# WangXinyan940/openmm-chargeflux

Measured on AMD Instinct MI355X. Metric: ns/day + ms/force-eval, periodic charge-flux box, 1/2/4/8 MI355X, higher is better.
Workload: dtype f64; 1 GPU; C3: periodic flexible charge-flux water box, 96000 atoms, Ewald rc=1.0 nm tol=0.0001 (alpha 2.91842, kmax 31, K_half 113490), velocity Verlet dt=1 fs, fp64; atoms=96000, k_half=113490, handover=event, variants=0, kspace=grid (ES kernel W=13, pruned DFT), same k-set, parallelism=atom-decomposition x1

## Files before the change

include/chargeflux.h:

```cpp
#ifndef CHARGEFLUX_H_
#define CHARGEFLUX_H_

#include <stdint.h>

#ifdef __cplusplus
extern "C" {
#endif

#if defined(_WIN32)
#define CF_EXPORT __declspec(dllexport)
#else
#define CF_EXPORT __attribute__((visibility("default")))
#endif

#define CF_API_VERSION 4

#define CF_OK 0
#define CF_ERR_INVALID -1
#define CF_ERR_HIP -2
#define CF_ERR_STATE -3
#define CF_ERR_NOMEM -4

#define CF_ONE_4PI_EPS0 138.935456
#define CF_ONE_4PI_EPS0_CODATA2018 138.93545764438198
// ... 26 lines not shown

typedef struct cf_options {
    int32_t device;
    void* stream;
    int32_t rank;
    int32_t world_size;
    int32_t kspace_algo;
    int32_t grid_width;
    int32_t precision;
    int32_t handover;
    int32_t pair_list;
    int32_t variants;
    int32_t list_capacity;
    int32_t reserved[1];
} cf_options;

#define CF_PRECISION_DOUBLE 0
#define CF_PRECISION_MIXED 1

#define CF_HANDOVER_EVENT 0
#define CF_HANDOVER_MEMORY 1

#define CF_PAIR_LIST_AUTO 0
#define CF_PAIR_LIST_CLUSTER 1
#define CF_PAIR_LIST_ATOM_HALF 2
#define CF_PAIR_LIST_FULL 3

#define CF_VARIANT_GEMM_DFT 1
#define CF_VARIANT_VECTOR_SPREAD 2
#define CF_VARIANT_MFMA_SPREAD 4
#define CF_VARIANT_INTERP1 8
#define CF_VARIANT_INTERP2 16
#define CF_VARIANT_BLOCK_ROUNDS(r) (((r) & 15) << 8)

#define CF_INCLUDE_FORCES 1
#define CF_INCLUDE_ENERGY 2

typedef struct cf_handle cf_handle;

CF_EXPORT int cf_api_version(void);
CF_EXPORT const char* cf_last_error(void);

CF_EXPORT int cf_create(const cf_params* params, const cf_options* options, cf_handle** out);
CF_EXPORT int cf_destroy(cf_handle* h);

CF_EXPORT int cf_get_ewald_params(const cf_handle* h, double* alpha, int32_t kmax[3]);
CF_EXPORT int cf_get_grid_shape(const cf_handle* h, int32_t ng[3], int32_t* width);
CF_EXPORT int cf_get_owned_range(const cf_handle* h, int32_t* lo, int32_t* hi);
CF_EXPORT int cf_partition(const cf_params* params, int32_t world_size, int32_t rank, int32_t* lo, int32_t* hi);

CF_EXPORT int cf_set_neighbor_skin(cf_handle* h, double skin);
CF_EXPORT int cf_update_parameters(cf_handle* h, const cf_params* params);
CF_EXPORT int cf_get_pair_list(const cf_handle* h, int32_t* kind);
CF_EXPORT int cf_get_neighbor_stats(const cf_handle* h, int64_t* builds, int64_t* evaluations);
#define CF_FALLBACK_WINDOW 1
#define CF_FALLBACK_LIST 2
#define CF_FALLBACK_FIXED_POINT 4
CF_EXPORT int cf_get_fallback_stats(const cf_handle* h, int64_t* half_list_fallbacks, int64_t* rows_rescanned,
                                    int32_t* reasons);

#define CF_GUARD_CELL_BOUNDS 1
#define CF_GUARD_CLUSTER_TABLE 2
#define CF_GUARD_LIST_ENTRY 4
#define CF_GUARD_GRID_BINS 8
#define CF_GUARD_NEIGHBOR 16
#define CF_GUARD_ATOM_INDEX 32
// ... 42 lines not shown
```

openmm-chargeflux_amd/csrc/cf_api.hip:

```cpp
#include <hip/hip_runtime.h>

#include <algorithm>
#include <cmath>
#include <cstring>
#include <exception>
#include <numeric>
#include <stdexcept>
#include <string>
#include <vector>

#include "cf_internal.h"

enum Phase { PH_FLUX, PH_PREP, PH_CELLS, PH_NLIST, PH_TABLES, PH_SFAC, PH_COEFFS, PH_FORCE, PH_DIRECT,
             PH_ASSEMBLE, PH_ENERGY, PH_GSORT, PH_GSPREAD, PH_GDFTF, PH_GDFTI, PH_GINTERP, PH_EXCL, PH_COUNT };
static const char* kPhaseNames[PH_COUNT] = {"flux_terms", "atoms_prep", "cell_sort", "neighbor_list",
                                            "kspace_tables", "kspace_sfac", "kspace_coeffs", "kspace_force",
                                            "direct_pairs", "assemble", "energy", "grid_sort", "grid_spread",
                                            "grid_dft_fwd", "grid_dft_inv", "grid_interp", "direct_excl"};
constexpr int kMaxTimed = 8192;

static void graph_forget(cf_handle* H);
static void graph_invalidate(cf_handle* H);
struct GraphCache;
static GraphCache* graph_active(cf_handle* H);
// ... 408 lines not shown
        if (!p || !out) fail(CF_ERR_INVALID, "null argument");
        const int n = p->num_particles;
        if (n <= 0) fail(CF_ERR_INVALID, "num_particles must be > 0");
        if (!p->charges || !p->sigmas || !p->epsilons) fail(CF_ERR_INVALID, "particle arrays are null");
        cf_options o;
        std::memset(&o, 0, sizeof(o));
        if (opt) o = *opt;
        int world = o.world_size <= 1 ? 1 : o.world_size;
        if (o.rank < 0 || o.rank >= world) fail(CF_ERR_INVALID, "rank out of range");

        int ndev = 0;
        check_hip(hipGetDeviceCount(&ndev), "hipGetDeviceCount");
        if (ndev <= 0) fail(CF_ERR_HIP, "no HIP device available");
        if (o.device < 0 || o.device >= ndev) fail(CF_ERR_INVALID, "device ordinal out of range");
        check_hip(hipSetDevice(o.device), "hipSetDevice");

        H = new cf_handle();
        cf::Handle& h = H->h;
        h.n = n;
        h.device = o.device;
        h.rank = o.rank;
        h.world = world;
        if (o.kspace_algo < 0 || o.kspace_algo > 2) fail(CF_ERR_INVALID, "kspace_algo must be 0, 1 or 2");
        if (o.grid_width != 0 && (o.grid_width < 4 || o.grid_width > 16))
            fail(CF_ERR_INVALID, "grid_width must be 0 (default) or in [4, 16]");
        if (o.precision != CF_PRECISION_DOUBLE && o.precision != CF_PRECISION_MIXED)
            fail(CF_ERR_INVALID, "precision must be CF_PRECISION_DOUBLE or CF_PRECISION_MIXED");
        h.mixed = o.precision == CF_PRECISION_MIXED;
        if (o.handover != CF_HANDOVER_EVENT && o.handover != CF_HANDOVER_MEMORY)
            fail(CF_ERR_INVALID, "handover must be CF_HANDOVER_EVENT or CF_HANDOVER_MEMORY");
        if (o.pair_list < CF_PAIR_LIST_AUTO || o.pair_list > CF_PAIR_LIST_FULL)
            fail(CF_ERR_INVALID, "pair_list must be one of CF_PAIR_LIST_AUTO, _CLUSTER, _ATOM_HALF, _FULL "
                                 "(the octant list of API 3 was removed in API 4)");
        if (o.variants & ~(0x1F | (15 << 8))) fail(CF_ERR_INVALID, "unknown bits in variants");
        if (o.list_capacity < 0) fail(CF_ERR_INVALID, "list_capacity must be >= 0");
        h.handover_memory = o.handover == CF_HANDOVER_MEMORY;
        h.pair_list = o.pair_list;
        h.variants = o.variants;
        h.list_capacity = o.list_capacity;
        h.kspace_algo = o.kspace_algo;
        h.stream = (hipStream_t)o.stream;

        std::vector<double> q0;
        std::vector<double2> lj;
        parse_particles(p, q0, lj);

        const int B = p->num_flux_bonds, A = p->num_flux_angles, W = p->num_flux_waters;
        const int T = B + A + W;
        std::vector<int4> tidx;
        std::vector<double> tpar;
        std::vector<std::vector<int>> term_atoms;
        parse_terms(p, tidx, tpar, &term_atoms);
        H->topo_terms = tidx;
        h.nb = B; h.na = A; h.nw = W; h.nterms = T;
        h.nslots_dq = 2 * B + 3 * A + 3 * W;
        h.nd = 4 * B + 9 * A + 9 * W;
        std::vector<int> slot_atom(h.nslots_dq);
        {
            int s = 0;
            for (int t = 0; t < T; t++)
                for (int a : term_atoms[t]) slot_atom[s++] = a;
        }
        std::vector<int> qs(n + 1, 0), qslot(h.nslots_dq);
        for (int s = 0; s < h.nslots_dq; s++) qs[slot_atom[s] + 1]++;
        for (int i = 0; i < n; i++) qs[i + 1] += qs[i];
        {
            std::vector<int> fill(qs.begin(), qs.end() - 1);
// ... 372 lines not shown
    const bool reusable = h.pbc && h.skin > 0 && h.list_valid && s_call == h.list_skin &&
                          h.list_L[0] == h.box_L[0] && h.list_L[1] == h.box_L[1] && h.list_L[2] == h.box_L[2] &&
                          h.list_T[0] == h.box_t[0] && h.list_T[1] == h.box_t[1] && h.list_T[2] == h.box_t[2];
    if (h.pbc && !reusable) {
        h.list_skin = s_call;
        set_cells(H, h.box_L);
        h.list_valid = h.skin > 0;
        std::copy(h.box_L, h.box_L + 3, h.list_L);
        std::copy(h.box_t, h.box_t + 3, h.list_T);
    }
    h.n_evals++;
    return reusable;
}

static void launch_begin(cf_handle* H, const double* pos_dev, int flags, bool reusable) {
    cf::Handle& h = H->h;
    const int forces = flags & CF_INCLUDE_FORCES, energy = flags & CF_INCLUDE_ENERGY;
    { Timed t(H, PH_FLUX); cf::launch_flux_terms(h, pos_dev); }
    { Timed t(H, PH_PREP); cf::launch_atoms_prep(h, pos_dev, reusable); }
    if (h.pbc) {
        {
            Timed t(H, PH_CELLS);
            if (!reusable) cf::launch_force_rebuild(h);
            cf::launch_cell_sort(h, pos_dev);
        }
        if (h.hi > h.lo) { Timed t(H, PH_NLIST); cf::launch_nlist(h, pos_dev); }
        if ((forces || energy) && h.hi > h.lo) {
            if (h.kspace_algo == 0) {
                { Timed t(H, PH_TABLES); cf::launch_kspace_tables(h, pos_dev); }
                { Timed t(H, PH_SFAC); cf::launch_kspace_sfac(h); }
            } else if (h.kspace_algo == 2) {
                { Timed t(H, PH_GSORT); cf::launch_grid_sort(h, pos_dev); }
                { Timed t(H, PH_GSPREAD); cf::launch_grid_spread(h); }
                { Timed t(H, PH_GDFTF); cf::launch_grid_dft_fwd(h); }
            } else {
                Timed t(H, PH_SFAC);
                cf::launch_kspace_direct_sfac(h, pos_dev);
            }
        } else if (forces || energy) {
            int64_t cnt = 0;
            double* buf = cf::kspace_reduce_buffer(h, &cnt);
            cf::launch_zero(h, buf, cnt);
            if (h.kspace_algo == 1) cf::launch_kspace_kvec(h);
        }
    }
}

static void launch_direct(cf_handle* H) {
    cf::Handle& h = H->h;
    if (h.hi <= h.lo) return;
    const int flags = h.pending_flags;
    const int forces = flags & CF_INCLUDE_FORCES, energy = flags & CF_INCLUDE_ENERGY;
    if (h.pbc) {
        { Timed t(H, PH_DIRECT); cf::launch_direct(h, H->pos_pending, forces); }
        { Timed t(H, PH_EXCL); cf::launch_direct_finish(h, H->pos_pending, forces); }
    } else {
        Timed t(H, PH_DIRECT);
        cf::launch_nopbc(h, H->pos_pending, forces, energy);
    }
}

static void launch_end(cf_handle* H, int flags, double* forces_dev, double* energy_dev) {
    cf::Handle& h = H->h;
    const int forces = flags & CF_INCLUDE_FORCES, energy = flags & CF_INCLUDE_ENERGY;
    const double* pos = H->pos_pending;
    if (h.pbc && (forces || energy) && (h.hi > h.lo || h.rank == 0)) {
        Timed t(H, PH_COEFFS);
// ... 103 lines not shown
        (void)hipGraphDestroy(graph);
        check_hip(e, "hipGraphInstantiate");
        g->exec[seg] = ex;
        g->key[seg] = k;
        g->rec_split[seg] = h.rec_split;
        g->captures++;
    } else {
        h.rec_split = g->rec_split[seg];
        g->replays++;
    }
    check_hip(hipGraphLaunch(g->exec[seg], h.stream), "hipGraphLaunch");
}

extern "C" {
static GraphKey make_key(const cf::Handle& h, const void* pos, void* frc, void* ene, int flags, bool reusable,
                         const double* box9) {
    GraphKey k;
    k.pos = pos; k.frc = frc; k.ene = ene; k.flags = flags; k.reusable = reusable;
    k.epoch = h.alloc_epoch;
    if (h.pbc && box9) std::memcpy(k.box, box9, sizeof(k.box));
    return k;
}

static bool overlap_ok(const cf::Handle& h, int flags) {
    return h.overlap && h.aux && h.world == 1 && h.pbc && h.kspace_algo == 2 && h.hi > h.lo &&
           (flags & (CF_INCLUDE_FORCES | CF_INCLUDE_ENERGY));
}

static void launch_prologue(cf_handle* H, const double* pos_dev, bool reusable) {
    cf::Handle& h = H->h;
    { Timed t(H, PH_FLUX); cf::launch_flux_terms(h, pos_dev); }
    { Timed t(H, PH_PREP); cf::launch_atoms_prep(h, pos_dev, reusable); }
}
static void launch_direct_chain(cf_handle* H, const double* pos_dev, int flags, bool reusable) {
    cf::Handle& h = H->h;
    {
        Timed t(H, PH_CELLS);
        if (!reusable) cf::launch_force_rebuild(h);
        cf::launch_cell_sort(h, pos_dev);
    }
    { Timed t(H, PH_NLIST); cf::launch_nlist(h, pos_dev); }
    h.pending_flags = flags;
    launch_direct(H);
    h.pending_flags = -1;
}
static void launch_rec_fwd(cf_handle* H, const double* pos_dev) {
    cf::Handle& h = H->h;
    { Timed t(H, PH_GSORT); cf::launch_grid_sort(h, pos_dev); }
    { Timed t(H, PH_GSPREAD); cf::launch_grid_spread(h); }
    { Timed t(H, PH_GDFTF); cf::launch_grid_dft_fwd(h); }
}
static void launch_rec_end(cf_handle* H, int flags) {
    cf::Handle& h = H->h;
    { Timed t(H, PH_COEFFS); cf::launch_grid_coeffs(h, flags & CF_INCLUDE_ENERGY, (flags & CF_INCLUDE_FORCES) != 0); }
    if (flags & CF_INCLUDE_FORCES) {
        { Timed t(H, PH_GDFTI); cf::launch_grid_dft_inv(h); }
        { Timed t(H, PH_GINTERP); cf::launch_grid_interp(h, true); }
    }
}
}
template <class F>
static void on_aux(cf_handle* H, GraphCache* g, int seg, const GraphKey& k, F&& launches) {
    cf::Handle& h = H->h;
    const hipStream_t main = h.stream;
    h.stream = h.aux;
    try {
        run_segment(H, g, seg, k, launches);
    } catch (...) {
        h.stream = main;
        throw;
    }
    h.stream = main;
}
extern "C" {
static void fork_aux(cf::Handle& h) {
    check_hip(hipEventRecord(h.ev_fork, h.stream), "hipEventRecord (fork)");
    check_hip(hipStreamWaitEvent(h.aux, h.ev_fork, 0), "hipStreamWaitEvent (fork)");
}
static void wait_fork(cf::Handle& h) {
    check_hip(hipStreamWaitValue64(h.aux, h.sync_flag, ++h.sync_seq, hipStreamWaitValueGte, ~0ull),
              "hipStreamWaitValue64 (fork)");
}
static void join_post(cf::Handle& h) {
// ... 40 lines not shown
    size_t nd = 0;
    check_hip(hipStreamGetCaptureInfo_v2(cap, &st, &id, &graph, &deps, &nd), "hipStreamGetCaptureInfo_v2");
    if (st != hipStreamCaptureStatusActive || !graph) fail(CF_ERR_STATE, "capture_event_wait: stream is not capturing");
    std::vector<hipGraphNode_t> dep(deps, deps + nd);
    hipGraphNode_t w = nullptr;
    check_hip(hipGraphAddEventWaitNode(&w, graph, dep.empty() ? nullptr : dep.data(), dep.size(), ev),
              "hipGraphAddEventWaitNode");
    check_hip(hipStreamUpdateCaptureDependencies(cap, &w, 1, hipStreamSetCaptureDependencies),
              "hipStreamUpdateCaptureDependencies");
}

static void launch_full(cf_handle* H, const double* pos_dev, int flags, bool reusable, double* forces_dev,
                        double* energy_dev, GraphCache* g, const double* box9) {
    cf::Handle& h = H->h;
    struct Restore {
        cf::Handle& h; hipStream_t s;
        ~Restore() { h.pending_flags = -1; h.stream = s; }
    } restore{h, h.stream};
    if (!overlap_ok(h, flags)) {
        auto one = [&] {
            h.rec_split = false;
            h.pending_flags = flags;
            launch_begin(H, pos_dev, flags, reusable);
            launch_direct(H);
            h.pending_flags = -1;
            launch_end(H, flags, forces_dev, energy_dev);
        };
        run_segment(H, g, SEG_FULL, make_key(h, pos_dev, forces_dev, energy_dev, flags, reusable, box9), one);
        return;
    }
    const int forces = flags & CF_INCLUDE_FORCES, energy = flags & CF_INCLUDE_ENERGY;
    const GraphKey key = make_key(h, pos_dev, nullptr, nullptr, flags, reusable, box9);
    auto rec = [&] {
        launch_rec_fwd(H, pos_dev);
        launch_rec_end(H, flags);
    };
    auto dch = [&] { launch_direct_chain(H, pos_dev, flags, reusable); };
    if (h.handover_memory) {
        SyncGuard sync_guard{h};
        run_segment(H, g, SEG_PRO, key, [&] {
            launch_prologue(H, pos_dev, reusable);
            cf::launch_signal(h, h.sync_flag);
            rec();
        });
        wait_fork(h);
        on_aux(H, g, SEG_DCH, key, [&] {
            dch();
            cf::launch_signal(h, h.sync_flag + 1);
        });
        join_wait(h);
    } else {
        launch_prologue(H, pos_dev, reusable);
        fork_aux(h);
        on_aux(H, g, SEG_DCH, key, dch);
        join_post(h);
        if (g) {
            const GraphKey key_rec = make_key(h, pos_dev, forces_dev, energy_dev, flags, reusable, box9);
            run_segment(H, g, SEG_REC, key_rec, [&] {
                rec();
                capture_event_wait(h.stream, h.ev_join);
                h.rec_split = forces != 0;
                cf::launch_assemble_energy(h, (forces && forces_dev) ? forces_dev : nullptr, energy, energy_dev);
            });
            h.rec_split = forces != 0;
            return;
        }
        run_segment(H, g, SEG_REC, key, rec);
        join_wait(h);
    }
    h.rec_split = forces != 0;
    Timed t(H, PH_ENERGY);
    cf::launch_assemble_energy(h, (forces && forces_dev) ? forces_dev : nullptr, energy, energy_dev);
}

static bool split_overlap_ok(cf_handle* H, int flags) {
    const cf::Handle& h = H->h;
    return h.overlap && h.aux && h.world > 1 && h.pbc && h.kspace_algo == 2 && h.hi > h.lo &&
           (flags & (CF_INCLUDE_FORCES | CF_INCLUDE_ENERGY));
}

static void launch_begin_split(cf_handle* H, const double* pos_dev, int flags, bool reusable, GraphCache* g,
                               const double* box9) {
    cf::Handle& h = H->h;
    const GraphKey key = make_key(h, pos_dev, nullptr, nullptr, flags, reusable, box9);
    if (h.handover_memory) {
        SyncGuard sync_guard{h};
        run_segment(H, g, SEG_PRO, key, [&] {
            launch_prologue(H, pos_dev, reusable);
            cf::launch_signal(h, h.sync_flag);
            launch_rec_fwd(H, pos_dev);
        });
        wait_fork(h);
        try {
            on_aux(H, g, SEG_DCH, key, [&] {
                launch_direct_chain(H, pos_dev, flags, reusable);
                cf::launch_signal(h, h.sync_flag + 1);
            });
        } catch (...) {
            h.pending_flags = -1;
            throw;
        }
        return;
    }
    run_segment(H, g, SEG_PRO, key, [&] { launch_prologue(H, pos_dev, reusable); });
    fork_aux(h);
    try {
        on_aux(H, g, SEG_DCH, key, [&] { launch_direct_chain(H, pos_dev, flags, reusable); });
    } catch (...) {
        h.pending_flags = -1;
        throw;
    }
    join_post(h);
    run_segment(H, g, SEG_RFWD, key, [&] { launch_rec_fwd(H, pos_dev); });
}

static void launch_end_split(cf_handle* H, int flags, double* forces_dev, double* energy_dev, GraphCache* g,
                             const double* box9) {
    cf::Handle& h = H->h;
    const int forces = flags & CF_INCLUDE_FORCES, energy = flags & CF_INCLUDE_ENERGY;
    SyncGuard sync_guard{h};
    run_segment(H, g, SEG_REND, make_key(h, H->pos_pending, nullptr, nullptr, flags, false, box9),
                [&] { launch_rec_end(H, flags); });
    join_wait(h);
    h.rec_split = forces != 0;
    {
        Timed t(H, PH_ENERGY);
        cf::launch_assemble_energy(h, (forces && forces_dev) ? forces_dev : nullptr, energy, energy_dev);
    }
}

static void ensure_aux(cf_handle* H) {
    cf::Handle& h = H->h;
    if (h.aux || !h.overlap || !h.pbc || h.kspace_algo != 2) return;
    check_hip(hipStreamCreateWithFlags(&h.aux, hipStreamNonBlocking), "hipStreamCreate (second stream)");
    const unsigned evf = hipEventDisableTiming | hipEventDisableSystemFence;
    check_hip(hipEventCreateWithFlags(&h.ev_fork, evf), "hipEventCreate");
    check_hip(hipEventCreateWithFlags(&h.ev_join, evf), "hipEventCreate");
    if (h.handover_memory && !h.sync_flag) {
        int can_wait = 0;
        if (hipDeviceGetAttribute(&can_wait, hipDeviceAttributeCanUseStreamWaitValue, h.device) != hipSuccess ||
            !can_wait) {
            h.handover_memory = false;
        } else {
            h.sync_flag = dalloc<unsigned long long>(H, 2);
            check_hip(hipMemsetAsync(h.sync_flag, 0, 2 * sizeof(unsigned long long), h.aux), "sync flag init");
            check_hip(hipStreamSynchronize(h.aux), "sync flag init");
// ... 311 lines not shown
```

openmm-chargeflux_amd/csrc/cf_internal.h:

```cpp
#pragma once

#include <hip/hip_runtime.h>
#include <stdint.h>

#include <string>
#include <vector>

#include "../../include/chargeflux.h"

namespace cf {

constexpr double kPi = 3.14159265358979323846;

struct KGeom {
    int KX = 0, KY = 0, KZ = 0;
    int NY = 0;
    int NYB = 0;
    int NYP = 0;
    int NYB4 = 0;
    int NMT = 0;
    int NZP = 0;
    int NB = 0;
    int CSW = 0;
    __host__ __device__ int nslots() const { return KX * NYP; }
// ... 180 lines not shown
    int sk_nchunk = 0;
    double* erfc_tab = nullptr;
    double erfc_scale = 0; int erfc_m = 0;
    double erfc_scale_f = 0; int erfc_m_f = 0;
    float* erfc_tab_f = nullptr;
    double* terms_dev = nullptr;
    double* e_part = nullptr;
    double* energy_dev = nullptr;
    int* e_ticket = nullptr;
    int pending_flags = -1;
    bool direct_done = false;
    double box_L[3] = {0, 0, 0};
    double box_t[3] = {0, 0, 0};
    bool tric = false;
};

std::vector<double> erfc_table(double xmax, double* scale, int* m);
std::vector<float> erfc_table_f(double xmax, double* scale, int* m);
std::vector<double> erfc_table_deg(double xmax, int deg, double width, int max_m, double* scale, int* m);
void launch_flux_terms(Handle& h, const double* pos);
void launch_atoms_prep(Handle& h, const double* pos, bool skin_check);
void launch_cell_sort(Handle& h, const double* pos);
void launch_force_rebuild(Handle& h);
void launch_zero(Handle& h, double* p, int64_t n);
void launch_nlist(Handle& h, const double* pos);
void launch_cluster_list(Handle& h);
void launch_pairs_cluster(Handle& h, const double* pos, int include_forces);
void launch_cluster_table(Handle& h);
void launch_direct(Handle& h, const double* pos, int include_forces);
void launch_direct_finish(Handle& h, const double* pos, int include_forces);
void launch_recip_add(Handle& h);
void launch_nopbc(Handle& h, const double* pos, int include_forces, int include_energy);
void launch_signal(Handle& h, unsigned long long* flag);
void launch_assemble_energy(Handle& h, double* forces_out, int include_energy, double* energy_out);

void kspace_plan(Handle& h);
size_t kspace_alloc_bytes(const Handle& h);
void launch_kspace_tables(Handle& h, const double* pos);
void launch_kspace_sfac(Handle& h);
double* kspace_reduce_buffer(Handle& h, int64_t* count);
void launch_kspace_coeffs(Handle& h, int include_energy);
void launch_kspace_force(Handle& h, const double* pos);

void launch_kspace_kvec(Handle& h);
void launch_kspace_direct_sfac(Handle& h, const double* pos);
void launch_kspace_direct_coeffs(Handle& h, int include_energy);
void launch_kspace_direct_force(Handle& h, const double* pos);

void grid_plan(Handle& h, int width, double sigma);
void grid_tables(const Handle& h, std::vector<double2> tw[3], std::vector<double2> tw8[3], std::vector<double> deconv[3]);
void launch_grid_sort(Handle& h, const double* pos);
void launch_grid_spread(Handle& h);
void launch_grid_dft_fwd(Handle& h);
double* grid_reduce_buffer(Handle& h, int64_t* count);
void launch_grid_coeffs(Handle& h, int include_energy, bool inverse_follows);
void launch_grid_dft_inv(Handle& h);
void launch_grid_interp(Handle& h, bool split = false);

void launch_om_gather(Handle& h, const void* posq, const void* corr, int posq_kind, const int* atom_index,
                      double* pos);
void launch_om_scatter(Handle& h, const int* atom_index, const double* frc, int padded, long long* fbuf,
                       const double* ene, void* ebuf, int energy_kind);

void check_hip(hipError_t e, const char* what);

#if defined(__HIP_DEVICE_COMPILE__)
#define CF_LDS_UNPAIRED __attribute__((target("no-load-store-opt")))
#else
#define CF_LDS_UNPAIRED
#endif

__device__ __forceinline__ double rsqrt_fp64(double r2) {
    double y = __builtin_amdgcn_rsq(r2);
    return y * fma(-0.5 * r2 * y, y, 1.5);
}

__device__ __forceinline__ double fma3(double a, double b, double c) {
    double d;
    asm("v_fma_f64 %0, %1, %2, %3" : "=v"(d) : "v"(a), "v"(b), "s"(c));
    return d;
}

__device__ __forceinline__ double exp_nonpos(double y) {
    const double k = rint(y * 1.4426950408889634);
    double r = fma(-k, 6.93147180369123816490e-01, y);
    r = fma(-k, 1.90821492927058770002e-10, r);
// ... 143 lines not shown
```

openmm-chargeflux_amd/csrc/cf_kernels_core.hip:

```cpp
#include <algorithm>
#include <type_traits>

#include "cf_pair.h"

namespace cf {


__device__ __forceinline__ long dqdx_start(int t, int nb, int na) {
    const int b = min(t, nb), an = max(0, min(t, nb + na) - nb), w = max(0, t - nb - na);
    return 3L * (4L * b + 9L * an + 9L * w);
}

__global__ void __launch_bounds__(256) k_flux_terms(int nterms, int nb, int na, const int4* __restrict__ tidx,
                                                    const double* __restrict__ tpar, const double* __restrict__ pos,
                                                    double3 L, double3 T, int pbc, double* __restrict__ dq_slot,
                                                    double* __restrict__ dqdx) {
    __shared__ double st[256 * 27];
    const int t0 = blockIdx.x * blockDim.x;
    const int t = t0 + threadIdx.x;
    const long base = dqdx_start(t0, nb, na);
    if (t < nterms) {
        int4 ti = tidx[t];
        const double* p = tpar + 5 * t;
        double* o = st + (dqdx_start(t, nb, na) - base);
// ... 1582 lines not shown
        if (ty) hipLaunchKernelGGL((k_pairs<16, true>), dim3(nblk((int64_t)a.nlr * 16, 256)), dim3(256), 0, h.stream, a);
        else hipLaunchKernelGGL((k_pairs<16, false>), dim3(nblk((int64_t)a.nlr * 16, 256)), dim3(256), 0, h.stream, a);
    }
}

void launch_direct_finish(Handle& h, const double* pos, int include_forces) {
    DirectArgs a = direct_args(h, pos, include_forces);
    hipLaunchKernelGGL(k_excl, dim3(nblk(a.nlr, 256)), dim3(256), 0, h.stream, a);
}

void launch_recip_add(Handle& h) {
    int nown = h.hi - h.lo;
    int nparts = h.kspace_algo == 0 ? h.fp.nparts() : 1;
    hipLaunchKernelGGL(k_recip_add, dim3(nblk(nown, 256)), dim3(256), 0, h.stream, h.lo, nown, nparts, h.t_part,
                       h.dedq, h.f_part);
}

void launch_nopbc(Handle& h, const double* pos, int include_forces, int include_energy) {
    int nown = h.hi - h.lo;
    hipLaunchKernelGGL(k_nopbc, dim3(nblk(nown, kNopbcTile)), dim3(kNopbcTile), 0, h.stream, h.n, h.lo, h.hi,
                       include_forces, include_energy, h.ke, pos, h.q, h.lj, h.ex_start, h.ex_list, h.dedq, h.f_part,
                       h.e_atom);
}

__global__ void k_signal(unsigned long long* __restrict__ flag) {
    if (threadIdx.x == 0) __hip_atomic_fetch_add(flag, 1ull, __ATOMIC_RELEASE, __HIP_MEMORY_SCOPE_SYSTEM);
}

void launch_signal(Handle& h, unsigned long long* flag) {
    hipLaunchKernelGGL(k_signal, dim3(1), dim3(64), 0, h.stream, flag);
    check_hip(hipPeekAtLastError(), "k_signal launch");
}

void launch_assemble_energy(Handle& h, double* forces_out, int include_energy, double* energy_out) {
    const int nown = std::max(0, h.hi - h.lo);
    int nrec = (h.pbc && include_energy && h.rank == 0) ? h.e_rec_nblk : 0;
    const int per = h.block_rounds() > 0 ? std::min(8, h.block_rounds()) : std::max(1, std::min(8, nown / (kEChunk * 512)));
    const int nparts = std::max(1, nblk(nown, kEChunk * per));
    hipLaunchKernelGGL(k_assemble_energy, dim3(nparts), dim3(kEChunk), 0, h.stream, h.lo, h.hi, h.ccsr_start,
                       h.ccsr_ent, h.dedq, h.dqdx, h.f_part, forces_out, h.rec_split ? h.dedq_rec : nullptr,
                       h.rec_split ? reinterpret_cast<const double4*>(h.f_rec) : nullptr,
                       make_double3(h.gp.ng[0] / h.box_L[0], h.gp.ng[1] / h.box_L[1], h.gp.ng[2] / h.box_L[2]), h.e_atom, h.e_part, h.e_rec_part, nrec, h.pbc,
                       h.terms_dev, energy_out, h.energy_dev, h.e_ticket + kTicketEnergy, h.skin_flag, h.g_xrange,
                       h.half ? h.half_flag : nullptr, h.n_fallback_dev, per, h.err_dev, h.err_host_dev);
}

}
```

openmm-chargeflux_amd/csrc/cf_kernels_grid.hip:

```cpp
#include <algorithm>
#include <cstdlib>
#include <cmath>
#include <utility>
#include <vector>

#include "cf_internal.h"

namespace cf {

static inline int nblk(int64_t n, int b) { return (int)((n + b - 1) / b); }

typedef double v2d __attribute__((ext_vector_type(2)));
typedef float v2f __attribute__((ext_vector_type(2)));

__device__ __forceinline__ int wave_id() { return __builtin_amdgcn_readfirstlane(threadIdx.x >> 6); }

__device__ __forceinline__ void es_tap(double t, double hw_inv, double beta, double& v, double& dv) {
    const double z = t * hw_inv;
    const double u = 1.0 - z * z;
    if (u > 0.0) {
        const double rs = rsqrt_fp64(u);
        v = exp_nonpos(beta * (u * rs - 1.0));
        dv = v * beta * z * rs * hw_inv;
    } else {
// ... 854 lines not shown
    double3 rec;
    double cst, one_4a2;
    const double *dx, *dy, *dz;
    double* e_part;
};

constexpr int kD8Seq = 64, kD8BC = 8;
constexpr int kDft8Mt[] = {4, 8, 9, 16, 17};

__device__ __forceinline__ v2d mul_i(v2d v) { return v2d{-v.y, v.x}; }

__device__ __forceinline__ void dft8(const v2d (&x)[8], v2d (&y)[8]) {
    const double c = 0.70710678118654752440;
    const v2d e0 = x[0] + x[4], e1 = x[0] - x[4], e2 = x[2] + x[6], e3 = x[2] - x[6];
    const v2d o0 = x[1] + x[5], o1 = x[1] - x[5], o2 = x[3] + x[7], o3 = x[3] - x[7];
    const v2d E0 = e0 + e2, E2 = e0 - e2, E1 = e1 + mul_i(e3), E3 = e1 - mul_i(e3);
    const v2d O0 = o0 + o2, O2 = o0 - o2, O1 = o1 + mul_i(o3), O3 = o1 - mul_i(o3);
    const v2d wO1 = v2d{c * (O1.x - O1.y), c * (O1.x + O1.y)};
    const v2d w3O3 = v2d{-c * (O3.x + O3.y), c * (O3.x - O3.y)};
    const v2d iO2 = mul_i(O2);
    y[0] = E0 + O0; y[4] = E0 - O0;
    y[1] = E1 + wO1; y[5] = E1 - wO1;
    y[2] = E2 + iO2; y[6] = E2 - iO2;
    y[3] = E3 + w3O3; y[7] = E3 - w3O3;
}

__device__ __forceinline__ void cmac(v2d& acc, v2d y, double2 t) {
    acc.x = fma(y.x, t.x, acc.x);
    acc.x = fma(-y.y, t.y, acc.x);
    acc.y = fma(y.x, t.y, acc.y);
    acc.y = fma(y.y, t.x, acc.y);
}

template <int MT, bool CIN, int SEQ, bool COEF = false>
__global__ void __launch_bounds__(8 * SEQ) k_g_dft8_fwd(Dft8 d, const double2* __restrict__ twist,
                                                        const double2* __restrict__ tq, Coef cf = Coef{}) {
    constexpr int NR = CIN ? 8 : 5, SP = SEQ + 1, NT = 8 * SEQ;
    extern __shared__ v2d sm8[];
    v2d* sY = sm8;
    v2d* stw = sm8 + kD8BC * NR * SP;
    const int s0 = blockIdx.x * SEQ;
    if (d.xmode == 1 && d.xr &&
        !x_range_in_slab(s0 / d.xdiv, min(s0 + SEQ - 1, d.nseq - 1) / d.xdiv, d.xr, d.W, d.ngx))
        return;
    const int tid = threadIdx.x, lane = tid & 63;
    const int sq = lane % SEQ, r = wave_id() * (64 / SEQ) + lane / SEQ;
    for (int e = tid; e < 8 * d.Q; e += NT) stw[e] = reinterpret_cast<const v2d*>(twist)[e];
    const int sl = CIN ? (tid % SEQ) : (tid >> 3), bl = CIN ? (tid / SEQ) : (tid & 7);
    const int si = s0 + sl;
    const bool sok = si < d.nseq;
    const long ibase = sok ? (long)(si / d.sdiv) * d.s1 + (long)(si % d.sdiv) * d.s0 : 0;
    v2d xn[8];
    auto load = [&](int bc) {
        const bool ok = sok && bc + bl < d.Q;
#pragma unroll
        for (int a = 0; a < 8; a++) {
            const int n = d.Q * a + bc + bl;
            const bool oka = ok && (d.xmode != 2 || x_in_slab(n, d.xr, d.W, d.ngx));
            if constexpr (CIN) {
                const v2d v = reinterpret_cast<const v2d*>(d.in)[oka ? ibase + n * d.sn : 0];
                xn[a] = oka ? v : v2d{0.0, 0.0};
            } else {
                const double v = reinterpret_cast<const double*>(d.in)[oka ? ibase + n * d.sn : 0];
                xn[a] = v2d{oka ? v : 0.0, 0.0};
            }
        }
    };
// ... 26 lines not shown
            for (int t = 0; t < MT; t++) cmac(acc[t], yt, tqb[b * MT + t]);
        }
        __syncthreads();
    }
    const int s = s0 + sq;
    if constexpr (!COEF) {
        if (s >= d.nseq) return;
        const long base = (long)(s / d.sdiv) * d.c1 + (long)(s % d.sdiv) * d.c0;
        const int cnt = d.rc[r], j0 = d.rj[r];
#pragma unroll
        for (int t = 0; t < MT; t++)
            if (t < cnt) reinterpret_cast<v2d*>(d.out)[base + (long)(j0 + 8 * t) * d.cj] = acc[t];
    } else {
        __shared__ double red[8 * SEQ / 64];
        double e = 0;
        if (s < d.nseq) {
            const long base = (long)(s / d.sdiv) * d.c1 + (long)(s % d.sdiv) * d.c0;
            const int cnt = d.rc[r], j0 = d.rj[r];
            const int nz = s % cf.KZ, ny = s / cf.KZ - (cf.KY - 1);
            const double ky = ny * cf.rec.y, kz = nz * cf.rec.z;
            const double wz = nz > 0 ? 2.0 : 1.0;
            const double Dyz = cf.dy[abs(ny)] * cf.dz[nz];
#pragma unroll
            for (int t = 0; t < MT; t++) {
                if (t < cnt) {
                    const int j = j0 + 8 * t, nx = j - (cf.KX - 1);
                    const double kx = nx * cf.rec.x;
                    const double k2 = kx * kx + ky * ky + kz * kz;
                    const double a = k2 > 0 ? exp(-k2 * 0.25 * cf.one_4a2) / k2 : 0.0;
                    const double D = cf.dx[abs(nx)] * Dyz;
                    const double sr = acc[t].x * D, si = acc[t].y * D;
                    e += 0.5 * wz * cf.cst * a * (sr * sr + si * si);
                    const double c = wz * cf.cst * a * D;
                    reinterpret_cast<v2d*>(d.out)[base + (long)j * d.cj] = v2d{c * sr, -c * si};
                }
            }
        }
#pragma unroll
        for (int m = 32; m >= 1; m >>= 1) e += __shfl_xor(e, m);
        if (lane == 0) red[wave_id()] = e;
        __syncthreads();
        if (tid == 0) {
            double tot = 0;
#pragma unroll
            for (int w = 0; w < 8 * SEQ / 64; w++) tot += red[w];
            cf.e_part[blockIdx.x] = tot;
        }
    }
}

constexpr int kZR = 8;
constexpr int kZIR = 16;

template <int MT, int NB, bool GF = false>
__global__ void __launch_bounds__(64 * NB) k_g_dft8_zfwd(Dft8 d, const double2* __restrict__ twist,
                                                         const double2* __restrict__ tq) {
    extern __shared__ v2d sm8[];
    constexpr int R = kZR;
    const int Q = d.Q;
    v2d* sY = sm8;
    v2d* stw = sm8 + R * Q * 5;
    v2d* sO = stw + 8 * Q;
    const int s0 = blockIdx.x * R;
    if (d.xmode == 1 && d.xr &&
        !x_range_in_slab(s0 / d.xdiv, min(s0 + R - 1, d.nseq - 1) / d.xdiv, d.xr, d.W, d.ngx))
        return;
    const int tid = threadIdx.x;
    for (int e = tid; e < 8 * Q; e += 64 * NB) stw[e] = reinterpret_cast<const v2d*>(twist)[e];
    using GT = std::conditional_t<GF, float, double>;
    const GT* in = reinterpret_cast<const GT*>(d.in);
    for (int it = tid; it < R * Q; it += 64 * NB) {
        const int row = it / Q, b = it - row * Q;
        const int s = s0 + row;
        const bool ok = s < d.nseq;
        const long base = (long)(ok ? s : 0) * d.s1 + b;
        v2d x[8], y[8];
#pragma unroll
        for (int a = 0; a < 8; a++) {
            const double v = (double)in[base + (long)Q * a];
// ... 1066 lines not shown
    const long NYKZ = (long)NY * KZ;
    Dft8 d{};
    d.Q = p.ng[axis] / 8;
    for (int r = 0; r < 8; r++) { d.rj[r] = p.rj[axis][r]; d.rc[r] = p.rc[axis][r]; }
    d.xr = h.g_xrange; d.W = p.W; d.ngx = ngx;
    if (axis == 2) {
        d.nseq = ngx * ngy; d.sdiv = 1;
        d.s1 = ngz; d.s0 = 0; d.sn = 1;
        d.c1 = KZ; d.c0 = 0; d.cj = 1;
        d.xmode = 1; d.xdiv = ngy;
    } else if (axis == 1) {
        d.nseq = ngx * KZ; d.sdiv = KZ;
        d.s1 = (long)ngy * KZ; d.s0 = 1; d.sn = KZ;
        d.c1 = NYKZ; d.c0 = 1; d.cj = KZ;
        d.xmode = 1; d.xdiv = KZ;
    } else {
        d.nseq = (int)NYKZ; d.sdiv = (int)NYKZ;
        d.s1 = 0; d.s0 = 1; d.sn = NYKZ;
        d.c1 = 0; d.c0 = 1; d.cj = NYKZ;
        d.xmode = 2; d.xdiv = 1;
    }
    return d;
}

#define CF_D8_MT(MT_, CALL) \
    switch (MT_) {          \
        case 4: CALL(4); break;   \
        case 8: CALL(8); break;   \
        case 9: CALL(9); break;   \
        case 16: CALL(16); break; \
        default: CALL(17); break; \
    }

static void d8_fwd(Handle& h, int axis, const void* in, void* out, const Coef* cf = nullptr) {
    Dft8 d = d8_stage(h, axis);
    d.in = in; d.out = out;
    const int nb = nblk(d.nseq, kD8Seq);
    const double2* twist = h.g_tw8[axis];
    const double2* tq = twist + 8 * d.Q;
    const int J = d.rc[0] + d.rc[1] + d.rc[2] + d.rc[3] + d.rc[4] + d.rc[5] + d.rc[6] + d.rc[7];
    const size_t lds = (size_t)(kZR * d.Q * 5 + 8 * d.Q + kZR * J) * sizeof(double2);
    if (axis == 2 && lds <= 64 * 1024) {
        const dim3 g((unsigned)nblk(d.nseq, kZR));
#define CF_D8Z(MT_)                                                                                     \
    if (h.gp.grid_f32) hipLaunchKernelGGL((k_g_dft8_zfwd<MT_, 4, true>), g, dim3(256), lds, h.stream, d, twist, tq); \
    else hipLaunchKernelGGL((k_g_dft8_zfwd<MT_, 4, false>), g, dim3(256), lds, h.stream, d, twist, tq)
        CF_D8_MT(h.gp.mt[axis], CF_D8Z)
#undef CF_D8Z
        return;
    }
    const bool small = nb >= 128 && nb < 2048;
    const int seq = small ? 16 : 64;
    const dim3 grid((unsigned)nblk(d.nseq, seq));
    const size_t lds2 = (size_t)(kD8BC * (axis == 2 ? 5 : 8) * (seq + 1) + 8 * d.Q) * sizeof(double2);
    if (cf) {
        h.e_rec_nblk = (int)grid.x;
#define CF_D8FC_(MT_, SEQ_) \
    hipLaunchKernelGGL((k_g_dft8_fwd<MT_, true, SEQ_, true>), grid, dim3(8 * SEQ_), lds2, h.stream, d, twist, tq, *cf)
#define CF_D8FC(MT_) if (small) CF_D8FC_(MT_, 16); else CF_D8FC_(MT_, 64);
        CF_D8_MT(h.gp.mt[axis], CF_D8FC)
#undef CF_D8FC
#undef CF_D8FC_
        return;
    }
#define CF_D8F_(MT_, CIN_, SEQ_) \
    hipLaunchKernelGGL((k_g_dft8_fwd<MT_, CIN_, SEQ_>), grid, dim3(8 * SEQ_), lds2, h.stream, d, twist, tq)
#define CF_D8F(MT_)                                         \
    if (axis == 2) { if (small) CF_D8F_(MT_, false, 16); else CF_D8F_(MT_, false, 64); } \
    else { if (small) CF_D8F_(MT_, true, 16); else CF_D8F_(MT_, true, 64); }
    CF_D8_MT(h.gp.mt[axis], CF_D8F)
#undef CF_D8F
#undef CF_D8F_
}

static void d8_inv(Handle& h, int axis, const void* in, void* out, const Coef* cf = nullptr) {
    Dft8 d = d8_stage(h, axis);
    d.in = in; d.out = out;
    if (axis == 0) d.xmode = 0;
    const size_t lds = (size_t)(kZIR * d.Q * 4 + 8 * d.Q) * sizeof(double2);
    if (axis == 2 && lds <= 64 * 1024) {
        const double2* tw0 = h.g_tw8[axis];
        const double2* tq0 = tw0 + 8 * d.Q;
        const dim3 g((unsigned)nblk(d.nseq, kZIR));
#define CF_D8ZI(MT_)                                                                                    \
    if (h.gp.grid_f32) hipLaunchKernelGGL((k_g_dft8_zinv<MT_, 2, true>), g, dim3(128), lds, h.stream, d, tw0, tq0); \
    else hipLaunchKernelGGL((k_g_dft8_zinv<MT_, 2, false>), g, dim3(128), lds, h.stream, d, tw0, tq0)
        CF_D8_MT(h.gp.mt[axis], CF_D8ZI)
#undef CF_D8ZI
        return;
    }
    const int nb = nblk(d.nseq, kD8Seq), nchunks = (d.Q + kD8BC - 1) / kD8BC;
    const dim3 grid((unsigned)nb, (unsigned)std::max(1, std::min(nchunks, 2048 / nb)));
    const double2* twist = h.g_tw8[axis];
    const double2* tq = twist + 8 * d.Q;
    const size_t lds2 = (size_t)(kD8BC * 8 * (kD8Seq + 1) + 8 * d.Q + d.Q * h.gp.mt[axis]) * sizeof(double2);
    if (cf) {
        h.e_rec_nblk = (int)grid.x;
#define CF_D8IC(MT_) \
    hipLaunchKernelGGL((k_g_dft8_inv<MT_, false, kD8Seq, true>), grid, dim3(8 * kD8Seq), lds2, h.stream, d, twist, tq, *cf)
        CF_D8_MT(h.gp.mt[axis], CF_D8IC)
#undef CF_D8IC
        return;
    }
#define CF_D8I(MT_)                                                                                            \
    if (axis == 2) hipLaunchKernelGGL((k_g_dft8_inv<MT_, true, kD8Seq>), grid, dim3(8 * kD8Seq), lds2, h.stream, d, twist, tq); \
    else hipLaunchKernelGGL((k_g_dft8_inv<MT_, false, kD8Seq>), grid, dim3(8 * kD8Seq), lds2, h.stream, d, twist, tq)
    CF_D8_MT(h.gp.mt[axis], CF_D8I)
#undef CF_D8I
}

static bool coef_fused(const Handle& h) { return h.gp.dft8 && h.world == 1; }

static Coef coef_args(const Handle& h) {
    const GridPlan& p = h.gp;
    const double V = h.box_L[0] * h.box_L[1] * h.box_L[2];
    return Coef{p.KX, p.KY, p.KZ, recip_vec(h), 4.0 / V * kPi * h.ke, 1.0 / (h.alpha * h.alpha), h.g_deconv[0],
                h.g_deconv[1], h.g_deconv[2], h.e_rec_part};
}

void launch_grid_dft_fwd(Handle& h) {
    const GridPlan& p = h.gp;
    if (p.dft8) {
        d8_fwd(h, 2, h.g_grid, h.g_t1);
        d8_fwd(h, 1, h.g_t1, h.g_t2);
        if (coef_fused(h)) {
            const Coef cf = coef_args(h);
            d8_fwd(h, 0, h.g_t2, h.g_b, &cf);
        } else {
            d8_fwd(h, 0, h.g_t2, h.g_b);
        }
        return;
    }
    const int ngx = p.ng[0], ngy = p.ng[1], ngz = p.ng[2], KZ = p.KZ, NY = p.NY, NX = p.NX;
    const long NYKZ = (long)NY * KZ;
    const double2* tzh = h.g_tw[2] + (size_t)(KZ - 1) * ngz;
    cgemm<true, false>(h, CGemm{ngx * ngy, KZ, ngz, h.g_grid, ngz, 1, tzh, 1, 0, ngz, h.g_t1, KZ, 0, 1, KZ}, 1, ngy);
    cgemm<false, false>(h, CGemm{NY, ngx * KZ, ngy, h.g_tw[1], ngy, 1, h.g_t1, KZ, (long)ngy * KZ, 1, h.g_t2, KZ, NYKZ,
                                 1, KZ}, 2, KZ);
    cgemm<false, false>(h, CGemm{NX, (int)NYKZ, ngx, h.g_tw[0], ngx, 1, h.g_t2, NYKZ, 0, 1, h.g_b, NYKZ, 0, 1,
                                 (int)NYKZ}, 3);
}

double* grid_reduce_buffer(Handle& h, int64_t* count) {
    *count = (int64_t)2 * h.gp.NX * h.gp.NY * h.gp.KZ;
    return reinterpret_cast<double*>(h.g_b);
}

void launch_grid_coeffs(Handle& h, int include_energy, bool inverse_follows) {
    h.coef_inv = 0;
    if (coef_fused(h)) return;
    if (h.gp.dft8 && inverse_follows) {
        h.coef_inv = include_energy ? 2 : 1;
        return;
    }
    const GridPlan& p = h.gp;
    const double V = h.box_L[0] * h.box_L[1] * h.box_L[2];
    const double cst = 4.0 / V * kPi * h.ke;
    const int total = p.NX * p.NY * p.KZ;
    h.e_rec_nblk = nblk(total, 256);
    hipLaunchKernelGGL(k_g_coeffs, dim3(h.e_rec_nblk), dim3(256), 0, h.stream, p.KX, p.KY, p.KZ, recip_vec(h), cst,
                       1.0 / (h.alpha * h.alpha), h.g_deconv[0], h.g_deconv[1], h.g_deconv[2], h.g_b, h.e_rec_part,
                       include_energy);
}

void launch_grid_dft_inv(Handle& h) {
    const GridPlan& p = h.gp;
    if (p.dft8) {
        if (h.coef_inv) {
            Coef cf = coef_args(h);
            if (h.coef_inv == 1) cf.e_part = nullptr;
            h.coef_inv = 0;
            d8_inv(h, 0, h.g_b, h.g_t2, &cf);
        } else {
            d8_inv(h, 0, h.g_b, h.g_t2);
        }
        d8_inv(h, 1, h.g_t2, h.g_t1);
        d8_inv(h, 2, h.g_t1, h.g_grid);
        return;
    }
    const int ngx = p.ng[0], ngy = p.ng[1], ngz = p.ng[2], KZ = p.KZ, NY = p.NY, NX = p.NX;
    const long NYKZ = (long)NY * KZ;
    const double2* tzh = h.g_tw[2] + (size_t)(KZ - 1) * ngz;
    cgemm<false, false>(h, CGemm{ngx, (int)NYKZ, NX, h.g_tw[0], 1, ngx, h.g_b, NYKZ, 0, 1, h.g_t2, NYKZ, 0, 1,
                                 (int)NYKZ}, 1, 1);
    cgemm<false, false>(h, CGemm{ngy, ngx * KZ, NY, h.g_tw[1], 1, ngy, h.g_t2, KZ, NYKZ, 1, h.g_t1, KZ,
                                 (long)ngy * KZ, 1, KZ}, 2, KZ);
    cgemm<false, true>(h, CGemm{ngx * ngy, ngz, KZ, h.g_t1, KZ, 1, tzh, ngz, 0, 1, h.g_grid, ngz, 0, 1, ngz}, 1, ngy);
}

void launch_grid_interp(Handle& h, bool split) {
    const GridPlan& p = h.gp;
    const int3 ng = make_int3(p.ng[0], p.ng[1], p.ng[2]), nb = make_int3(p.nb[0], p.nb[1], p.nb[2]);
    const double3 gs = make_double3(p.ng[0] / h.box_L[0], p.ng[1] / h.box_L[1], p.ng[2] / h.box_L[2]);
    const size_t R = 7 + p.W;
#define CF_INTERP(W_)                                                                                               \
    hipLaunchKernelGGL(!p.interp2 ? k_g_interp<W_>                                                                 \
                       : (W_ <= 8 && p.interp4) ? (p.grid_f32 ? k_g_interp4<(W_ <= 8 ? W_ : 8), true, true>            \
                                                   : h.mixed ? k_g_interp4<(W_ <= 8 ? W_ : 8), true, false>            \
                                                             : k_g_interp4<(W_ <= 8 ? W_ : 8), false, false>)          \
                                                : k_g_interp2<W_>,                                                     \
                       dim3(p.nbins), dim3(kInterpThreads),                                                         \
// ... 10 lines not shown
```

openmm-chargeflux_amd/openmmcoul/_cabi.py:

```python
from __future__ import annotations

import ctypes as C
import os
import threading

_PKG_ROOT = os.path.dirname(os.path.dirname(os.path.abspath(__file__)))
LIB_PATH = os.path.join(_PKG_ROOT, "libchargeflux_hip.so")

CF_OK = 0
CF_ERR_INVALID = -1
CF_ERR_HIP = -2
CF_ERR_STATE = -3
CF_ERR_NOMEM = -4
CF_PRECISION_DOUBLE = 0
CF_PRECISION_MIXED = 1
CF_HANDOVER_EVENT = 0
CF_HANDOVER_MEMORY = 1
CF_PAIR_LIST_AUTO = 0
CF_PAIR_LIST_CLUSTER = 1
CF_PAIR_LIST_ATOM_HALF = 2
CF_PAIR_LIST_FULL = 3
CF_VARIANT_GEMM_DFT = 1
CF_VARIANT_VECTOR_SPREAD = 2
CF_VARIANT_MFMA_SPREAD = 4
CF_VARIANT_INTERP1 = 8
CF_VARIANT_INTERP2 = 16


def CF_VARIANT_BLOCK_ROUNDS(r: int) -> int:
    return (int(r) & 15) << 8


CF_GUARD_CELL_BOUNDS = 1
CF_GUARD_CLUSTER_TABLE = 2
CF_GUARD_LIST_ENTRY = 4
CF_GUARD_GRID_BINS = 8
CF_GUARD_NEIGHBOR = 16
CF_GUARD_ATOM_INDEX = 32
CF_GUARD_REBUILD_FLAG = 64
CF_POSQ_DOUBLE4 = 0
CF_POSQ_FLOAT4 = 1
CF_ENERGY_DOUBLE = 0
CF_ENERGY_FLOAT = 1
CF_INCLUDE_FORCES = 1
CF_INCLUDE_ENERGY = 2
ONE_4PI_EPS0 = 138.935456
ONE_4PI_EPS0_CODATA2018 = 138.93545764438198


class cf_params(C.Structure):
    _fields_ = [
        ("num_particles", C.c_int32),
        ("charges", C.POINTER(C.c_double)),
        ("sigmas", C.POINTER(C.c_double)),
        ("epsilons", C.POINTER(C.c_double)),
        ("num_exceptions", C.c_int32),
        ("exceptions", C.POINTER(C.c_int32)),
        ("num_flux_bonds", C.c_int32),
        ("flux_bond_idx", C.POINTER(C.c_int32)),
# ... 109 lines not shown
```

Before: 198.0 ns/day.

## Fuse first inverse x-stage DFT into coefficient-fused forward x-stage kernel

When forces are requested on a single device, the forward x-axis DFT8 kernel that applies the Ewald coefficients now keeps the scaled coefficients in registers and immediately runs the first inverse x-stage transform, writing the result in place into g_t2. The separate inverse x-stage launch is then skipped. This is meant to remove one full grid round trip through global memory and one kernel launch, at the cost of a heavier kernel with more registers and LDS traffic. It also adds an optional delay kernel variant and an opt-out flag, both off by default.

Result: no change. 199.9 ns/day, median of 4 (+0.9%).

```diff
diff --git a/include/chargeflux.h b/include/chargeflux.h
--- a/include/chargeflux.h
+++ b/include/chargeflux.h
@@ -82,6 +82,8 @@
 #define CF_VARIANT_INTERP1 8
 #define CF_VARIANT_INTERP2 16
 #define CF_VARIANT_BLOCK_ROUNDS(r) (((r) & 15) << 8)
+#define CF_VARIANT_XSTAGE_UNFUSED 32
+#define CF_VARIANT_AUX_DELAY 64
 
 #define CF_INCLUDE_FORCES 1
 #define CF_INCLUDE_ENERGY 2
diff --git a/openmm-chargeflux_amd/csrc/cf_api.hip b/openmm-chargeflux_amd/csrc/cf_api.hip
--- a/openmm-chargeflux_amd/csrc/cf_api.hip
+++ b/openmm-chargeflux_amd/csrc/cf_api.hip
@@ -464,7 +464,7 @@
         if (o.pair_list < CF_PAIR_LIST_AUTO || o.pair_list > CF_PAIR_LIST_FULL)
             fail(CF_ERR_INVALID, "pair_list must be one of CF_PAIR_LIST_AUTO, _CLUSTER, _ATOM_HALF, _FULL "
                                  "(the octant list of API 3 was removed in API 4)");
-        if (o.variants & ~(0x1F | (15 << 8))) fail(CF_ERR_INVALID, "unknown bits in variants");
+        if (o.variants & ~(0x1F | CF_VARIANT_XSTAGE_UNFUSED | CF_VARIANT_AUX_DELAY | (15 << 8))) fail(CF_ERR_INVALID, "unknown bits in variants");
         if (o.list_capacity < 0) fail(CF_ERR_INVALID, "list_capacity must be >= 0");
         h.handover_memory = o.handover == CF_HANDOVER_MEMORY;
         h.pair_list = o.pair_list;
@@ -903,7 +903,7 @@
             } else if (h.kspace_algo == 2) {
                 { Timed t(H, PH_GSORT); cf::launch_grid_sort(h, pos_dev); }
                 { Timed t(H, PH_GSPREAD); cf::launch_grid_spread(h); }
-                { Timed t(H, PH_GDFTF); cf::launch_grid_dft_fwd(h); }
+                { Timed t(H, PH_GDFTF); cf::launch_grid_dft_fwd(h, forces != 0); }
             } else {
                 Timed t(H, PH_SFAC);
                 cf::launch_kspace_direct_sfac(h, pos_dev);
@@ -1073,8 +1073,12 @@
     { Timed t(H, PH_FLUX); cf::launch_flux_terms(h, pos_dev); }
     { Timed t(H, PH_PREP); cf::launch_atoms_prep(h, pos_dev, reusable); }
 }
+static void aux_delay(cf::Handle& h) {
+    if (h.variants & CF_VARIANT_AUX_DELAY) cf::launch_delay(h);
+}
 static void launch_direct_chain(cf_handle* H, const double* pos_dev, int flags, bool reusable) {
     cf::Handle& h = H->h;
+    aux_delay(h);
     {
         Timed t(H, PH_CELLS);
         if (!reusable) cf::launch_force_rebuild(h);
@@ -1085,11 +1089,11 @@
     launch_direct(H);
     h.pending_flags = -1;
 }
-static void launch_rec_fwd(cf_handle* H, const double* pos_dev) {
+static void launch_rec_fwd(cf_handle* H, const double* pos_dev, int flags) {
     cf::Handle& h = H->h;
     { Timed t(H, PH_GSORT); cf::launch_grid_sort(h, pos_dev); }
     { Timed t(H, PH_GSPREAD); cf::launch_grid_spread(h); }
-    { Timed t(H, PH_GDFTF); cf::launch_grid_dft_fwd(h); }
+    { Timed t(H, PH_GDFTF); cf::launch_grid_dft_fwd(h, (flags & CF_INCLUDE_FORCES) != 0); }
 }
 static void launch_rec_end(cf_handle* H, int flags) {
     cf::Handle& h = H->h;
@@ -1196,7 +1200,7 @@
     const int forces = flags & CF_INCLUDE_FORCES, energy = flags & CF_INCLUDE_ENERGY;
     const GraphKey key = make_key(h, pos_dev, nullptr, nullptr, flags, reusable, box9);
     auto rec = [&] {
-        launch_rec_fwd(H, pos_dev);
+        launch_rec_fwd(H, pos_dev, flags);
         launch_rec_end(H, flags);
     };
     auto dch = [&] { launch_direct_chain(H, pos_dev, flags, reusable); };
@@ -1252,7 +1256,7 @@
         run_segment(H, g, SEG_PRO, key, [&] {
             launch_prologue(H, pos_dev, reusable);
             cf::launch_signal(h, h.sync_flag);
-            launch_rec_fwd(H, pos_dev);
+            launch_rec_fwd(H, pos_dev, flags);
         });
         wait_fork(h);
         try {
@@ -1275,7 +1279,7 @@
         throw;
     }
     join_post(h);
-    run_segment(H, g, SEG_RFWD, key, [&] { launch_rec_fwd(H, pos_dev); });
+    run_segment(H, g, SEG_RFWD, key, [&] { launch_rec_fwd(H, pos_dev, flags); });
 }
 
 static void launch_end_split(cf_handle* H, int flags, double* forces_dev, double* energy_dev, GraphCache* g,
diff --git a/openmm-chargeflux_amd/csrc/cf_internal.h b/openmm-chargeflux_amd/csrc/cf_internal.h
--- a/openmm-chargeflux_amd/csrc/cf_internal.h
+++ b/openmm-chargeflux_amd/csrc/cf_internal.h
@@ -236,6 +236,7 @@
 void launch_recip_add(Handle& h);
 void launch_nopbc(Handle& h, const double* pos, int include_forces, int include_energy);
 void launch_signal(Handle& h, unsigned long long* flag);
+void launch_delay(Handle& h);
 void launch_assemble_energy(Handle& h, double* forces_out, int include_energy, double* energy_out);
 
 void kspace_plan(Handle& h);
@@ -255,7 +256,7 @@
 void grid_tables(const Handle& h, std::vector<double2> tw[3], std::vector<double2> tw8[3], std::vector<double> deconv[3]);
 void launch_grid_sort(Handle& h, const double* pos);
 void launch_grid_spread(Handle& h);
-void launch_grid_dft_fwd(Handle& h);
+void launch_grid_dft_fwd(Handle& h, bool inverse_follows);
 double* grid_reduce_buffer(Handle& h, int64_t* count);
 void launch_grid_coeffs(Handle& h, int include_energy, bool inverse_follows);
 void launch_grid_dft_inv(Handle& h);
diff --git a/openmm-chargeflux_amd/csrc/cf_kernels_core.hip b/openmm-chargeflux_amd/csrc/cf_kernels_core.hip
--- a/openmm-chargeflux_amd/csrc/cf_kernels_core.hip
+++ b/openmm-chargeflux_amd/csrc/cf_kernels_core.hip
@@ -1638,6 +1638,21 @@
     check_hip(hipPeekAtLastError(), "k_signal launch");
 }
 
+constexpr int kDelayMaxRounds = 4096;
+__global__ void __launch_bounds__(64) k_delay(long long ticks) {
+    const long long t0 = wall_clock64();
+    for (int it = 0; it < kDelayMaxRounds; it++) {
+        if (wall_clock64() - t0 >= ticks) break;
+        __builtin_amdgcn_s_sleep(32);
+    }
+}
+
+void launch_delay(Handle& h) {
+    int khz = 0;
+    if (hipDeviceGetAttribute(&khz, hipDeviceAttributeWallClockRate, h.device) != hipSuccess || khz <= 0) khz = 100000;
+    hipLaunchKernelGGL(k_delay, dim3(1), dim3(64), 0, h.stream, (long long)khz * 300 / 1000);
+}
+
 void launch_assemble_energy(Handle& h, double* forces_out, int include_energy, double* energy_out) {
     const int nown = std::max(0, h.hi - h.lo);
     int nrec = (h.pbc && include_energy && h.rank == 0) ? h.e_rec_nblk : 0;
diff --git a/openmm-chargeflux_amd/csrc/cf_kernels_grid.hip b/openmm-chargeflux_amd/csrc/cf_kernels_grid.hip
--- a/openmm-chargeflux_amd/csrc/cf_kernels_grid.hip
+++ b/openmm-chargeflux_amd/csrc/cf_kernels_grid.hip
@@ -910,7 +910,7 @@
     acc.y = fma(y.y, t.x, acc.y);
 }
 
-template <int MT, bool CIN, int SEQ, bool COEF = false>
+template <int MT, bool CIN, int SEQ, bool COEF = false, bool XINV = false>
 __global__ void __launch_bounds__(8 * SEQ) k_g_dft8_fwd(Dft8 d, const double2* __restrict__ twist,
                                                         const double2* __restrict__ tq, Coef cf = Coef{}) {
     constexpr int NR = CIN ? 8 : 5, SP = SEQ + 1, NT = 8 * SEQ;
@@ -1003,9 +1003,16 @@
                     const double sr = acc[t].x * D, si = acc[t].y * D;
                     e += 0.5 * wz * cf.cst * a * (sr * sr + si * si);
                     const double c = wz * cf.cst * a * D;
-                    reinterpret_cast<v2d*>(d.out)[base + (long)j * d.cj] = v2d{c * sr, -c * si};
+                    if constexpr (XINV) acc[t] = v2d{c * sr, -c * si};
+                    else reinterpret_cast<v2d*>(d.out)[base + (long)j * d.cj] = v2d{c * sr, -c * si};
                 }
             }
+        }
+        if constexpr (XINV) {
+            const int cnt = s < d.nseq ? d.rc[r] : 0;
+#pragma unroll
+            for (int t = 0; t < MT; t++)
+                if (t >= cnt) acc[t] = v2d{0.0, 0.0};
         }
 #pragma unroll
         for (int m = 32; m >= 1; m >>= 1) e += __shfl_xor(e, m);
@@ -1016,6 +1023,35 @@
 #pragma unroll
             for (int w = 0; w < 8 * SEQ / 64; w++) tot += red[w];
             cf.e_part[blockIdx.x] = tot;
+        }
+        if constexpr (XINV) {
+            static_assert(CIN, "the x stage reads complex input");
+            v2d* sZ = sY;
+            for (int bc = 0; bc < d.Q; bc += kD8BC) {
+                const int nb = min(kD8BC, d.Q - bc);
+                const v2d* twr = stw + r * d.Q + bc;
+                const double2* tqb = tq + (long)bc * MT;
+#pragma unroll 2
+                for (int b = 0; b < nb; b++) {
+                    v2d z = v2d{0.0, 0.0}, zt = v2d{0.0, 0.0};
+#pragma unroll
+                    for (int t = 0; t < MT; t++) cmac(z, acc[t], tqb[b * MT + t]);
+                    const v2d tw = twr[b];
+                    cmac(zt, z, make_double2(tw.x, tw.y));
+                    sZ[(b * 8 + r) * SP + sq] = zt;
+                }
+                __syncthreads();
+                if (sok && bl < nb) {
+                    v2d z[8], x[8];
+#pragma unroll
+                    for (int q = 0; q < 8; q++) z[q] = sZ[(bl * 8 + q) * SP + sl];
+                    dft8(z, x);
+#pragma unroll
+                    for (int a = 0; a < 8; a++)
+                        reinterpret_cast<v2d*>(d.out)[ibase + (long)(d.Q * a + bc + bl) * d.sn] = x[a];
+                }
+                __syncthreads();
+            }
         }
     }
 }
@@ -2148,7 +2184,7 @@
         default: CALL(17); break; \
     }
 
-static void d8_fwd(Handle& h, int axis, const void* in, void* out, const Coef* cf = nullptr) {
+static void d8_fwd(Handle& h, int axis, const void* in, void* out, const Coef* cf = nullptr, bool xinv = false) {
     Dft8 d = d8_stage(h, axis);
     d.in = in; d.out = out;
     const int nb = nblk(d.nseq, kD8Seq);
@@ -2171,12 +2207,14 @@
     const size_t lds2 = (size_t)(kD8BC * (axis == 2 ? 5 : 8) * (seq + 1) + 8 * d.Q) * sizeof(double2);
     if (cf) {
         h.e_rec_nblk = (int)grid.x;
-#define CF_D8FC_(MT_, SEQ_) \
-    hipLaunchKernelGGL((k_g_dft8_fwd<MT_, true, SEQ_, true>), grid, dim3(8 * SEQ_), lds2, h.stream, d, twist, tq, *cf)
-#define CF_D8FC(MT_) if (small) CF_D8FC_(MT_, 16); else CF_D8FC_(MT_, 64);
+#define CF_D8FC__(MT_, SEQ_, XINV_) \
+    hipLaunchKernelGGL((k_g_dft8_fwd<MT_, true, SEQ_, true, XINV_>), grid, dim3(8 * SEQ_), lds2, h.stream, d, twist, tq, *cf)
+#define CF_D8FC_(MT_, SEQ_) if (xinv) CF_D8FC__(MT_, SEQ_, true); else CF_D8FC__(MT_, SEQ_, false)
+#define CF_D8FC(MT_) if (small) { CF_D8FC_(MT_, 16); } else { CF_D8FC_(MT_, 64); }
         CF_D8_MT(h.gp.mt[axis], CF_D8FC)
 #undef CF_D8FC
 #undef CF_D8FC_
+#undef CF_D8FC__
         return;
     }
 #define CF_D8F_(MT_, CIN_, SEQ_) \
@@ -2227,6 +2265,8 @@
 
 static bool coef_fused(const Handle& h) { return h.gp.dft8 && h.world == 1; }
 
+static bool x_fused(const Handle& h) { return coef_fused(h) && !(h.variants & CF_VARIANT_XSTAGE_UNFUSED); }
+
 static Coef coef_args(const Handle& h) {
     const GridPlan& p = h.gp;
     const double V = h.box_L[0] * h.box_L[1] * h.box_L[2];
@@ -2234,14 +2274,15 @@
                 h.g_deconv[1], h.g_deconv[2], h.e_rec_part};
 }
 
-void launch_grid_dft_fwd(Handle& h) {
+void launch_grid_dft_fwd(Handle& h, bool inverse_follows) {
     const GridPlan& p = h.gp;
     if (p.dft8) {
         d8_fwd(h, 2, h.g_grid, h.g_t1);
         d8_fwd(h, 1, h.g_t1, h.g_t2);
         if (coef_fused(h)) {
             const Coef cf = coef_args(h);
-            d8_fwd(h, 0, h.g_t2, h.g_b, &cf);
+            if (inverse_follows && x_fused(h)) d8_fwd(h, 0, h.g_t2, h.g_t2, &cf, true);
+            else d8_fwd(h, 0, h.g_t2, h.g_b, &cf);
         } else {
             d8_fwd(h, 0, h.g_t2, h.g_b);
         }
@@ -2282,7 +2323,8 @@
 void launch_grid_dft_inv(Handle& h) {
     const GridPlan& p = h.gp;
     if (p.dft8) {
-        if (h.coef_inv) {
+        if (x_fused(h)) {
+        } else if (h.coef_inv) {
             Coef cf = coef_args(h);
             if (h.coef_inv == 1) cf.e_part = nullptr;
             h.coef_inv = 0;
diff --git a/openmm-chargeflux_amd/openmmcoul/_cabi.py b/openmm-chargeflux_amd/openmmcoul/_cabi.py
--- a/openmm-chargeflux_amd/openmmcoul/_cabi.py
+++ b/openmm-chargeflux_amd/openmmcoul/_cabi.py
@@ -25,6 +25,8 @@
 CF_VARIANT_MFMA_SPREAD = 4
 CF_VARIANT_INTERP1 = 8
 CF_VARIANT_INTERP2 = 16
+CF_VARIANT_XSTAGE_UNFUSED = 32
+CF_VARIANT_AUX_DELAY = 64
 
 
 def CF_VARIANT_BLOCK_ROUNDS(r: int) -> int:
```
